# antarcticrainforest/seabreeze_param

Measured on AMD Instinct MI355X. Metric: grid-points/sec for sea_breeze_diag on N2560x1920 global grid; achieved HBM GB/s, higher is better.
Workload: dtype f64; 1 GPU; seabreeze_diag generic flavour, N1280 (2560x1920) global grid, nz=56, fp64 (BASELINE.json configs[2]); stream=torch's current stream (torch and the library share one HIP runtime), plan_cache=stored, nx=2560, ny=1920, nz=56, search_halo=16, parallelism=latband1, variant=default, comm=none, multi_rank_rccl=unmeasured on hardware so far (one GPU per box in the build pool)

## Files before the change

seabreeze_param_amd/csrc/sb_capi.hip:

```cpp
#include "../../include/seabreeze_hip.h"
#include "sb_launch.hpp"

#include <dlfcn.h>
#include <rccl/rccl.h>

#include <algorithm>
#include <chrono>
#include <cmath>
#include <condition_variable>
#include <functional>
#include <mutex>
#include <thread>
#include <cstdio>
#include <cstdlib>
#include <cstring>
#include <string>
#include <vector>

namespace {

thread_local std::string g_err;

struct DevBuf {
    void *p = nullptr;
    size_t cap = 0;
};

}

class HostPool {
  public:
    explicit HostPool(int n) {
        for (int i = 0; i < n; ++i) workers_.emplace_back([this] { loop(); });
    }
    ~HostPool() {
        { std::lock_guard<std::mutex> g(m_); quit_ = true; }
        cv_.notify_all();
        for (auto &t : workers_) t.join();
    }
    void run(int n, const std::function<void(int)> &fn) {
        if (n <= 0) return;
        {
            std::lock_guard<std::mutex> g(m_);
            fn_ = &fn; next_ = 0; total_ = n; done_ = 0;
            ++epoch_;
        }
        cv_.notify_all();
        work();
        std::unique_lock<std::mutex> lk(m_);
        done_cv_.wait(lk, [this] { return done_ == total_; });
        fn_ = nullptr;
    }
    int threads() const { return (int)workers_.size() + 1; }

  private:
    void work() {
        for (;;) {
            int i;
            const std::function<void(int)> *f;
            {
                std::lock_guard<std::mutex> g(m_);
                if (!fn_ || next_ >= total_) return;
                i = next_++;
                f = fn_;
            }
            (*f)(i);
            {
                std::lock_guard<std::mutex> g(m_);
                if (++done_ == total_) done_cv_.notify_all();
            }
        }
    }
    void loop() {
        unsigned long seen = 0;
        for (;;) {
            {
                std::unique_lock<std::mutex> lk(m_);
                cv_.wait(lk, [&] { return quit_ || epoch_ != seen; });
                if (quit_) return;
                seen = epoch_;
            }
            work();
        }
    }
    std::vector<std::thread> workers_;
    std::mutex m_;
    std::condition_variable cv_, done_cv_;
    const std::function<void(int)> *fn_ = nullptr;
    int next_ = 0, total_ = 0, done_ = 0;
    unsigned long epoch_ = 0;
    bool quit_ = false;
};

enum { SB_TICKET_WORDS = 2 };

struct DiagStream {
    bool active = false;
    HostPool *pool = nullptr;
    int nlons = 0, nlats = 0, esz = 0;
    DevBuf z, sd, cdist, ws, wd, thc, p1, theta, v, u, out;
    void *pin_in[2] = {nullptr, nullptr};
    void *pin_out[2] = {nullptr, nullptr};
    size_t pin_in_cap = 0, pin_out_cap = 0;
    hipEvent_t ev_in[2] = {nullptr, nullptr}, ev_out[2] = {nullptr, nullptr};
    long steps = 0;
    double host_copy_s = 0.0, enqueue_s = 0.0, wait_s = 0.0;
};

struct sb_ctx {
    int device = 0;
    hipStream_t stream = nullptr;
    std::string err;
    int radius_hint = 16;
    int ncu = 256;
    int ncu_dev = 256;
    int static_sigma = 0;
    bool stats_valid = false;
    int host_depth = 0;
    int no_fold = 0;
    int no_plan_cache = 0;
    int no_wide_strip = 0;
    int band_late_wind = 0;
    const void *stats_sigma = nullptr;
    int stats_dims[4] = {0, 0, 0, 0};
    int stats_ngathered = 0;
    int rep_launches = 0, rep_rccl = 0, rep_groups = 0, rep_copies = 0;
    DevBuf t0, bandbits, clsbits, tiles, vecs, nws, nwd, coastbits, tile_list, seg_list, stamps, jobcopy, plan;
    DevBuf umbits;
    int plan_key[8] = {0, 0, 0, 0, 0, 0, 0, 0};
    const void *plan_bits = nullptr;
    int call_seq = 0, plan_use = 0;
    bool segs_built = false;
    int tiles_n = 0, tiles_strip = -1, flag_parity = 0;
    int *last_flags = nullptr;
    Moments *partials = nullptr;
    unsigned int *ticket = nullptr;
    void *stats = nullptr;
    int *counters = nullptr;
    int *seg_count = nullptr;
    std::vector<unsigned char> dist_key, dist_hv;
    bool dist_ordered = false;
    double dist_maxstep = 0.0;
    hipStream_t dist_upload_stream = nullptr;
    std::vector<DevBuf> stage;
    Geo last_g{};
    int last_tiles = 0;
    bool have_last = false;
    const Moments *gathered = nullptr;
    int ngathered = 0;
    std::vector<hipEvent_t> prof_ev;
    std::vector<unsigned> prof_mask;
    int prof_calls = 0, prof_max = 0;
    hipStream_t aux_stream = nullptr;
    hipEvent_t ev_fork = nullptr, ev_join = nullptr, ev_mom = nullptr;
    Moments *band_moments_out = nullptr;
    int band_geo = 0;
    DevBuf band_mom;
    void *rccl_lib = nullptr;
    void *comm = nullptr;
    int rank = 0, nranks = 1;
    DiagStream ds;
};

namespace {

int fail(sb_ctx *c, int code, const std::string &msg) {
    if (c) c->err = msg; else g_err = msg;
    return code;
}

int hipfail(sb_ctx *c, hipError_t e, const char *what) {
    return fail(c, SB_ERR_HIP, std::string(what) + ": " + hipGetErrorString(e));
}

#define HIPCHK(c, call)                                         \
    do {                                                        \
        hipError_t e__ = (call);                                \
// ... 6 lines not shown
    b.p = nullptr;
    b.cap = 0;
    hipError_t e = hipMalloc(&b.p, bytes);
    if (e != hipSuccess) return fail(c, SB_ERR_ALLOC, std::string("hipMalloc: ") + hipGetErrorString(e));
    b.cap = bytes;
    return SB_OK;
}

template <typename T>
Geo make_geo(int nx, int ny, int h, int bnd, int rows) {
    Geo g;
    g.nx = nx; g.ny = ny; g.h = h;
    g.nxh = nx + 2 * h; g.nyh = ny + 2 * h;
    g.nw = (g.nxh + 63) / 64;
    g.bnd = bnd; g.rows = rows;
    g.band = 0;
    return g;
}

int pick_halo(const sb_ctx *c) {
    int r = c->radius_hint;
    if (r <= 8) return 8;
    if (r <= 16) return 16;
    if (r <= 24) return 24;
    return SB_MAX_LDS_HALO;
}

template <typename T>
static bool strip_kernel_runs(const sb_ctx *c, int nx, int rows) {
    const int H = pick_halo(c);
    int tx, ty;
    if (H > 16) return sizeof(T) == 4 && !c->no_wide_strip && sb_strip32_shape(nx, rows, &tx, &ty);
    return sb_strip_shape(nx, rows, &tx, &ty);
}

template <typename T>
static bool reuse_stats(const sb_ctx *c, const T *sigma, int nx, int ny, int halo) {
    return c->static_sigma && c->host_depth == 0 && c->stats_valid && c->stats_sigma == (const void *)sigma && c->stats_dims[0] == nx &&
           c->stats_dims[1] == ny && c->stats_dims[2] == halo && c->stats_dims[3] == (int)sizeof(T) &&
           c->stats_ngathered == (c->gathered ? c->ngathered : 0);
}

template <typename T>
int run_diag(sb_ctx *c, DiagJob<T> &job, hipStream_t st, int phases = 3) {
    const Geo &g = job.g;
    const size_t ncell = (size_t)g.nxh * g.nyh;
    const size_t nbits = (size_t)g.nyh * g.nw * sizeof(uint64_t);
    int rc;
    if ((rc = ensure(c, c->bandbits, nbits))) return rc;
    if ((rc = ensure(c, c->clsbits, nbits))) return rc;
    const int H = pick_halo(c);
    int txw, tyrows, tx, ty;
    const bool strip32 = H > 16 && sizeof(T) == 4 && !c->no_wide_strip && sb_strip32_shape(g.nx, g.rows, &tx, &ty);
    const bool strip = strip32 || (H <= 16 && sb_strip_shape(g.nx, g.rows, &tx, &ty));
    const int vb = strip32 ? 2 : 1;
    if (strip) { txw = 32; tyrows = 16; }
    else {
        sb_thc_tile_shape(H > 16 ? H : 24, &txw, &tyrows);
        tx = (g.nx + txw - 1) / txw; ty = (g.rows + tyrows - 1) / tyrows;
    }
    const int Hk = strip32 ? 32 : strip ? 16 : (H > 16 ? H : 24);
    const int ntile = strip ? tx * (ty + 2 * vb) : tx * ty;
    const int nflag = ntile + 2;
    if (c->tiles.cap < (size_t)2 * nflag * sizeof(int) || c->tiles_n != nflag || c->tiles_strip != (strip ? vb : 0)) {
        if ((rc = ensure(c, c->tiles, (size_t)2 * nflag * sizeof(int)))) return rc;
        HIPCHK(c, hipMemsetAsync(c->tiles.p, 0, (size_t)2 * nflag * sizeof(int), st));
        c->tiles_n = nflag;
        c->tiles_strip = strip ? vb : 0;
        c->flag_parity = 0;
    }
    int *flags_now = (int *)c->tiles.p + (size_t)c->flag_parity * nflag;
    int *flags_next = (int *)c->tiles.p + (size_t)(1 - c->flag_parity) * nflag;
    job.thc_ty = tyrows; job.thc_ntx = tx; job.thc_nty = ty;
    job.thc_txs = txw == 32 ? 5 : 6;
    job.strip = strip32 ? 2 : strip ? 1 : 0;
    if (strip) { job.tile_sx = ty + 2 * vb; job.tile_sy = 1; job.tile_off = vb; }
    else { job.tile_sx = 1; job.tile_sy = tx; job.tile_off = 0; }
    job.bandbits = (uint64_t *)c->bandbits.p;
    job.clsbits = (uint64_t *)c->clsbits.p;
    job.stats = (const T *)c->stats;
    job.tile_nnmax = flags_now;
    job.counters = flags_now + (size_t)ntile;
    job.ticket = (int *)c->ticket;
    job.next_flags = flags_next;
    job.next_flags_n = nflag;
    if ((rc = ensure(c, c->tile_list, ((size_t)ntile + (size_t)2 * c->ncu + 2) * sizeof(int)))) return rc;
    job.tile_pad = 2 * c->ncu;
    const size_t nseg = (size_t)g.nyh * g.nw;
    const size_t seg_cap = (nseg + SB_SEG_PARTS - 1) / SB_SEG_PARTS;
    if ((rc = ensure(c, c->seg_list, seg_cap * SB_SEG_PARTS * sizeof(SbSegEntry)))) return rc;
    job.tile_list = (int *)c->tile_list.p;
    job.seg_list = (SbSegEntry *)c->seg_list.p;
    job.seg_count = c->seg_count;
    job.seg_cap = (int)seg_cap;
    job.t0_fly = (job.flavour == SB_FLAVOUR_GENERIC) ? 1 : 0;
    const bool late_wind = c->band_late_wind && c->gathered && strip && job.t0_fly && !c->no_fold;
    job.wind_final = ((phases == 3 && !c->gathered) || late_wind) ? 1 : 0;
    job.nws = job.nwd = nullptr;
    if (!job.wind_final) {
        if ((rc = ensure(c, c->nws, (size_t)g.nx * g.ny * sizeof(T)))) return rc;
        if ((rc = ensure(c, c->nwd, (size_t)g.nx * g.ny * sizeof(T)))) return rc;
        job.nws = (T *)c->nws.p;
        job.nwd = (T *)c->nwd.p;
    }
    job.t0 = nullptr;
    if (!job.t0_fly) {
        if ((rc = ensure(c, c->t0, ncell * sizeof(T)))) return rc;
        job.t0 = (T *)c->t0.p;
    }
    if ((rc = ensure(c, c->jobcopy, sizeof(DiagJob<double>)))) return rc;
    job.self = (DiagJob<T> *)c->jobcopy.p;
    job.plan = nullptr; job.plan_gen = nullptr; job.call_id = 0; job.plan_use = 0; job.seg_trust = 0;
    job.moments_out = nullptr; job.stats_ticket = nullptr; job.strip_update = 0;
    if (strip) {
        const size_t need = 64 + (size_t)c->ncu * SB_PLAN_STRIDE;
        if (c->plan.cap < need) {
            if ((rc = ensure(c, c->plan, need))) return rc;
            HIPCHK(c, hipMemsetAsync(c->plan.p, 0, need, st));
            c->plan_bits = nullptr;
        }
        if (phases & 1) {
            if (c->call_seq == 0x7fffffff) {
                HIPCHK(c, hipMemsetAsync(c->plan.p, 0, need, st));
                c->call_seq = 0;
                c->plan_bits = nullptr;
            }
            ++c->call_seq;
            const int key[8] = {g.nx, g.ny, g.h, g.bnd, g.rows, c->ncu, tx, ty | (vb << 24)};
            c->plan_use = c->plan_bits == c->bandbits.p && std::memcmp(key, c->plan_key, sizeof(key)) == 0 ? 1 : 0;
            std::memcpy(c->plan_key, key, sizeof(key));
            c->plan_bits = c->bandbits.p;
        }
        job.plan = (char *)c->plan.p + 64;
        job.plan_gen = (int *)c->plan.p;
        job.call_id = c->call_seq;
        job.plan_use = c->no_plan_cache ? 0 : c->plan_use;
    } else if (phases & 1) c->plan_bits = nullptr;
    job.stamps = nullptr;
#ifdef SB_STAMPS
    if ((rc = ensure(c, c->stamps, (size_t)4096 * SB_NSTAMP * sizeof(long long)))) return rc;
    job.stamps = (long long *)c->stamps.p;
#endif
    SbLaunchCtx lc;
    lc.stream = st;
    lc.prof = nullptr;
    lc.prof_mask = nullptr;
    if (phases == 3 && c->prof_calls < c->prof_max) {
        lc.prof_mask = &c->prof_mask[(size_t)c->prof_calls];
        lc.prof = &c->prof_ev[(size_t)SB_PROF_EVENTS * c->prof_calls++];
    }
    lc.partials = c->partials; lc.stats = c->stats;
    lc.gathered = c->gathered; lc.ngathered = c->ngathered; lc.ncu = c->ncu;
    lc.moments_out = (phases == 1) ? c->band_moments_out : nullptr;
    lc.moments_event = (phases == 1 && c->nranks > 1) ? c->ev_mom : nullptr;
    lc.stats_ticket = (int *)c->ticket + 1;
    lc.phases = phases;
    lc.reuse_stats = reuse_stats<T>(c, job.sigma, g.nx, g.ny, g.h);
    lc.no_fold = c->no_fold != 0;
    const bool strip_folds = strip && job.t0_fly && !c->no_fold;
    lc.segs_stand = strip_folds && c->gathered && c->plan_use && c->segs_built && !c->no_plan_cache;
    job.fold = 0; job.fold_partials = nullptr; job.fold_nparts = 0; job.stats_out = nullptr;
    job.lists_stand = (strip_folds && !c->gathered && phases == 3 && c->plan_use && c->segs_built && !c->no_plan_cache) ? 1 : 0;
    job.gath = nullptr; job.ngath = 0;
    int launched = 0;
    lc.launches = &launched;
    if (phases == 3) c->rep_launches = c->rep_rccl = c->rep_groups = c->rep_copies = 0;
// ... 1333 lines not shown
```

seabreeze_param_amd/csrc/sb_device.hpp:

```cpp
#pragma once
#include <hip/hip_runtime.h>
#include <stdint.h>

#define SB_WAVE 64
#define SB_NSTAMP 32

enum { SB_FLAVOUR_GENERIC = 0, SB_FLAVOUR_WRAPPER = 1 };
enum { BND_WRAPPER = 0, BND_GLOBAL = 1, BND_HALO = 2 };

struct Moments {
    double n, mean, m2, mn, mx;
};

__host__ __device__ inline Moments moments_empty() {
    Moments m;
    m.n = 0.0; m.mean = 0.0; m.m2 = 0.0;
    m.mn = 1.0e308; m.mx = -1.0e308;
    return m;
}

__host__ __device__ inline Moments moments_merge(const Moments &a, const Moments &b) {
    if (b.n == 0.0) return a;
    if (a.n == 0.0) return b;
    Moments r;
// ... 104 lines not shown
        o.mx = __shfl_down(m.mx, off);
        m = moments_merge(m, o);
    }
    return m;
}

template <int NW>
__device__ __forceinline__ Moments block_merge_w(Moments m, Moments *wpart) {
    m = wave_merge(m);
    const int lane = threadIdx.x & 63, wv = threadIdx.x >> 6;
    __syncthreads();
    if (lane == 0) wpart[wv] = m;
    __syncthreads();
    Moments r = moments_empty();
    if (threadIdx.x < SB_WAVE) {
        if (threadIdx.x < NW) r = wpart[threadIdx.x];
        r = wave_merge(r);
    }
    return r;
}
__device__ __forceinline__ Moments block_merge(Moments m, Moments *wpart) {
    return block_merge_w<SB_STATS_NT / SB_WAVE>(m, wpart);
}

template <typename T>
__device__ __forceinline__ void sigmoid_scalars(const Moments &m, T *__restrict__ stats) {
    const T var = (T)m.m2;
    const T cnt = (T)m.n;
    stats[0] = T(2) / sqrt(var / cnt);
    stats[1] = ((T)m.mx - (T)m.mn) / T(4);
    stats[2] = (T)m.mean;
    stats[3] = var;
}

#endif

struct Geo {
    int nx, ny;
    int h;
    int nxh, nyh;
    int nw;
    int bnd;
    int rows;
    int band;
};
enum { GEO_BAND_EW = 1, GEO_BAND_SOUTH = 2, GEO_BAND_NORTH = 4 };

__device__ __forceinline__ bool sb_map_cell(const Geo &g, int xs, int ys, int &X, int &Y) {
    if (g.bnd == BND_HALO) {
        if (g.band & GEO_BAND_EW) {
            int m = xs % g.nx;
            xs = m < 0 ? m + g.nx : m;
        }
        if ((g.band & GEO_BAND_SOUTH) && ys < 0) ys = 0;
        if ((g.band & GEO_BAND_NORTH) && ys >= g.ny) ys = g.ny - 1;
        X = xs + g.h;
        Y = ys + g.h;
        return X >= 0 && X < g.nxh && Y >= 0 && Y < g.nyh;
    }
    int yy = ys < 0 ? 0 : (ys >= g.ny ? g.ny - 1 : ys);
    Y = yy;
    if (g.bnd == BND_WRAPPER) {
        int m = (xs + 1) % g.nx;
        if (m < 0) m += g.nx;
        X = (m < 1 ? 1 : m) - 1;
    } else {
        int m = xs % g.nx;
        if (m < 0) m += g.nx;
        X = m;
    }
    return true;
}

struct SbSegEntry {
    uint64_t word;
    uint32_t seg, pad;
};
#define SB_PLAN_SCHED 384
#define SB_PLAN_NQ 64
#define SB_PLAN_ENT_OFF 64
#define SB_PLAN_LIST_OFF (SB_PLAN_ENT_OFF + 8 * SB_PLAN_SCHED)
#define SB_PLAN_STRIDE (SB_PLAN_LIST_OFF + 2048 * SB_PLAN_NQ)
#define SB_SEG_PARTS 64

template <typename T>
struct DiagJob {
    Geo g;
    int nz;
    int flavour;
    int tn;
    int refresh;
    T target_plev, thr_wind, thr_dir, thr_ch, thr_thc, maxdist, fill;
    const T *p, *u, *v;
    const T *theta, *mask, *z, *sigma;
    int mask_ld;
    unsigned mask_off;
    int level_rule;
    T *ws, *wd, *thc, *sb_con;
    T *out;
    T *nws, *nwd;
    int *next_flags;
    int next_flags_n;
    int wind_final;
    int t0_fly;
    T *t0;
    uint64_t *bandbits;
    uint64_t *clsbits;
    const T *stats;
    int thc_ty, thc_ntx, thc_nty;
    int thc_txs;
    int tile_sx, tile_sy, tile_off;
    int strip;
    char *plan;
    int *plan_gen;
    int call_id;
    int plan_use;
    Moments *moments_out;
    int *stats_ticket;
    int strip_update;
    int seg_trust;
    int *tile_nnmax;
    int *ticket;
    int *tile_list;
    int tile_pad;
    SbSegEntry *seg_list;
    int *seg_count;
    int seg_cap;
    const Moments *gath;
    int ngath;
    int fold;
    int lists_stand;
    const Moments *fold_partials;
    int fold_nparts;
    T *stats_out;
    DiagJob<T> *self;
    int *counters;
    long long *stamps;
};

template <typename T>
struct StripJob {
    Geo g;
    const T *theta, *z, *sigma;
    const uint64_t *clsbits, *bandbits;
    T *thc;
    int *flags;
    int ntx, nty;
    int fold, fold_nparts, ngath, seg_cap;
    int lists_stand;
    int update;
    const T *stats;
    T *stats_out;
    const Moments *fold_partials, *gath;
    SbSegEntry *seg_list;
    int *seg_count;
    const DiagJob<T> *cold;
    char *plan;
    const int *plan_gen;
    int call_id, plan_use;
    long long *stamps;
};

__device__ __forceinline__ int sb_bit(const uint64_t *bits, int nw, int X, int Y) {
    return (int)((bits[(size_t)Y * nw + (X >> 6)] >> (X & 63)) & 1ull);
}

template <typename T>
__host__ __device__ inline T sb_modulo(T a, T p) {
    T r;
    if (p > T(0) && fabs(a) < p) r = a;
    else if (p > T(0) && a >= p && a < p + p) r = a - p;
    else r = fmod(a, p);
    if ((a < T(0)) != (p < T(0))) {
        if (r == T(0)) r = -r; else r += p;
    }
    return r;
}

template <typename T>
__device__ __forceinline__ T sb_logistic_of_neg(T y) {
    return T(1) / (T(1) + exp(y));
}
template <>
__device__ __forceinline__ double sb_logistic_of_neg<double>(double y) {
    y = fmin(fmax(y, -708.0), 700.0);
    const double n = __builtin_rint(y * 1.4426950408889634);
    double r = __builtin_fma(-n, 0.6931471805599453, y);
    r = __builtin_fma(-n, 2.3190468138462996e-17, r);
    const double r2 = r * r;
    double e = __builtin_fma(r2, 2.755731922398589e-07, 2.48015873015873e-05);
    double o = __builtin_fma(r2, 2.505210838544172e-08, 2.7557319223985893e-06);
    e = __builtin_fma(e, r2, 1.388888888888889e-03);   o = __builtin_fma(o, r2, 1.984126984126984e-04);
    e = __builtin_fma(e, r2, 4.1666666666666664e-02);  o = __builtin_fma(o, r2, 8.333333333333333e-03);
    e = __builtin_fma(e, r2, 0.5);                     o = __builtin_fma(o, r2, 1.6666666666666666e-01);
    e = __builtin_fma(e, r2, 1.0);                     o = __builtin_fma(o, r2, 1.0);
    const double p = __builtin_fma(o, r, e);
    const double x = 1.0 + ldexp(p, (int)n);
    double q = __builtin_amdgcn_rcp(x);
    q = __builtin_fma(q, __builtin_fma(-x, q, 1.0), q);
    q = __builtin_fma(q, __builtin_fma(-x, q, 1.0), q);
    return q;
}

template <typename T>
__device__ __forceinline__ T sb_t0(T theta, T z, T sigma, T sd, T r) {
// ... 49 lines not shown
```

seabreeze_param_amd/csrc/sb_diag_kernels.hip:

```cpp
#include "sb_device.hpp"
#include "sb_launch.hpp"
#include "sb_scan_body.hpp"

#define STATS_NT SB_STATS_NT

__device__ __forceinline__ Moments moments_from_shifted(double c, double s1, double s2, double mn, double mx,
                                                         int cnt) {
    Moments acc = moments_empty();
    if (cnt > 0) {
        acc.n = (double)cnt;
        acc.mean = c + s1 / acc.n;
        acc.m2 = s2 - s1 * s1 / acc.n;
        acc.mn = mn;
        acc.mx = mx;
    }
    return acc;
}

__device__ __forceinline__ void store_partial(Moments acc, Moments *wpart, Moments *__restrict__ partials) {
    acc = block_merge(acc, wpart);
    if (threadIdx.x == 0) partials[blockIdx.x] = acc;
}

template <typename T>
__global__ __launch_bounds__(STATS_NT) void k_stats(const T *__restrict__ ary, int nx, int ny, int ld,
                                                    size_t off0, Moments *__restrict__ partials, int *__restrict__ ticket,
                                                    T *__restrict__ stats, Moments *__restrict__ moments_out) {
    const unsigned n = (unsigned)nx * (unsigned)ny;
    const unsigned stride = gridDim.x * STATS_NT;
    const bool flat = (ld == nx);
    const double c = (double)ary[off0];
    double s1 = 0.0, s2 = 0.0, mn = 1.0e308, mx = -1.0e308;
    int cnt = 0;
    for (unsigned base = blockIdx.x * STATS_NT + threadIdx.x; base < n; base += 8 * stride) {
        double x[8];
#pragma unroll
        for (int q = 0; q < 8; ++q) {
            const unsigned i = base + q * stride;
            x[q] = c;
            if (i < n) {
                const size_t idx = flat ? (size_t)i : (size_t)(i / (unsigned)nx) * ld + (i % (unsigned)nx);
                x[q] = (double)ary[off0 + idx];
            }
        }
#pragma unroll
        for (int q = 0; q < 8; ++q) {
            if (base + q * stride < n) {
                const double d = x[q] - c;
                s1 += d;
                s2 += d * d;
                mn = x[q] < mn ? x[q] : mn;
                mx = x[q] > mx ? x[q] : mx;
                ++cnt;
            }
        }
    }
    __shared__ Moments wpart[STATS_NT / SB_WAVE];
    __shared__ int s_last;
    const Moments mine = block_merge(moments_from_shifted(c, s1, s2, mn, mx, cnt), wpart);
    if (threadIdx.x == 0) {
        double *dst = (double *)&partials[blockIdx.x];
        const double v[5] = {mine.n, mine.mean, mine.m2, mine.mn, mine.mx};
        static_assert(sizeof(Moments) == 5 * sizeof(double), "Moments is five doubles");
        for (int i = 0; i < 5; ++i) __hip_atomic_store(dst + i, v[i], __ATOMIC_RELAXED, __HIP_MEMORY_SCOPE_AGENT);
        asm volatile("s_waitcnt vmcnt(0)" ::: "memory");
        const int t = __hip_atomic_fetch_add(ticket, 1, __ATOMIC_RELAXED, __HIP_MEMORY_SCOPE_AGENT);
        s_last = t == (int)gridDim.x - 1 ? 1 : 0;
    }
    __syncthreads();
    if (!s_last) return;
    Moments m = moments_empty();
    for (int b = threadIdx.x; b < (int)gridDim.x; b += STATS_NT) {
        const double *src = (const double *)&partials[b];
        Moments o;
        o.n = __hip_atomic_load(src + 0, __ATOMIC_RELAXED, __HIP_MEMORY_SCOPE_AGENT);
        o.mean = __hip_atomic_load(src + 1, __ATOMIC_RELAXED, __HIP_MEMORY_SCOPE_AGENT);
        o.m2 = __hip_atomic_load(src + 2, __ATOMIC_RELAXED, __HIP_MEMORY_SCOPE_AGENT);
        o.mn = __hip_atomic_load(src + 3, __ATOMIC_RELAXED, __HIP_MEMORY_SCOPE_AGENT);
        o.mx = __hip_atomic_load(src + 4, __ATOMIC_RELAXED, __HIP_MEMORY_SCOPE_AGENT);
        m = moments_merge(m, o);
    }
    __syncthreads();
// ... 163 lines not shown
            const Moments o = partials[b];
            v.n += o.n; v.mean += o.mean; v.m2 += o.m2;
            v.mn = fmin(v.mn, o.mn); v.mx = fmax(v.mx, o.mx);
        }
        const Moments m = moments_of_shifted(c, block_total_shifted<PREP_NT / SB_WAVE>(v, wpart));
        if (tid == 0) {
            if (moments_out) *moments_out = m;
            else sigmoid_scalars<T>(m, stats);
        }
        return;
    }
    if (blockIdx.x == 1) {
        if (job.strip) return;
        const int ntiles = job.thc_ntx * job.thc_nty;
        int total;
        if (ntiles <= PREP_MAXCH * PREP_NT) {
            total = block_compact(ntiles, s_cnt, s_w, [&](int t) { return job.tile_nnmax[t] != 0; },
                                  [&](int rank, int t) { job.tile_list[1 + rank] = t; });
        } else {
            const int per = (ntiles + PREP_NT - 1) / PREP_NT;
            const int t0 = tid * per, t1 = min(t0 + per, ntiles);
            int cnt = 0;
            for (int t = t0; t < t1; ++t) cnt += job.tile_nnmax[t] != 0 ? 1 : 0;
            int at = block_excl_scan(cnt, s_w, total);
            for (int t = t0; t < t1; ++t)
                if (job.tile_nnmax[t] != 0) job.tile_list[1 + at++] = t;
        }
        if (tid == 0) job.tile_list[0] = total;
        for (int i = tid; i < job.tile_pad; i += PREP_NT) job.tile_list[1 + total + i] = -1;
        return;
    }
    const int part = (int)blockIdx.x - 2;
    const unsigned nseg = (unsigned)job.g.nyh * (unsigned)job.g.nw;
    const unsigned cap = (unsigned)job.seg_cap;
    const unsigned s0 = min((unsigned)part * cap, nseg), s1 = min(s0 + cap, nseg);
    SbSegEntry *list = job.seg_list + (size_t)part * cap;
    int total;
    if (cap <= (unsigned)(PREP_MAXCH * PREP_NT)) {
        total = block_compact((int)(s1 - s0), s_cnt, s_w, [&](int i) { return job.bandbits[s0 + (unsigned)i] != 0; },
                              [&](int rank, int i) {
                                  SbSegEntry e;
                                  e.word = job.bandbits[s0 + (unsigned)i]; e.seg = s0 + (unsigned)i; e.pad = 0;
                                  list[rank] = e;
                              });
    } else {
        const unsigned per = (cap + PREP_NT - 1) / PREP_NT;
        const unsigned a0 = min(s0 + (unsigned)tid * per, s1), a1 = min(a0 + per, s1);
        int cnt = 0;
        for (unsigned sg = a0; sg < a1; ++sg) cnt += job.bandbits[sg] != 0 ? 1 : 0;
        int at = block_excl_scan(cnt, s_w, total);
        for (unsigned sg = a0; sg < a1; ++sg) {
            const uint64_t w = job.bandbits[sg];
            if (w) { SbSegEntry e; e.word = w; e.seg = sg; e.pad = 0; list[at++] = e; }
        }
    }
    if (tid == 0) job.seg_count[part] = total;
}

#define WIND_NT 256

template <typename T, bool NTL>
__device__ __forceinline__ T sb_ld(const T *p) {
    if constexpr (NTL) return __builtin_nontemporal_load(p);
    else return *p;
}

template <typename T> struct WindCfg { static constexpr int UN = SB_WIND_UN, WGS = SB_WIND_WGS_PER_CU; };
template <> struct WindCfg<float> { static constexpr int UN = SB_WIND_UN_F32, WGS = SB_WIND_WGS_PER_CU_F32; };

#ifdef SB_STAMPS_WIND
#define SB_WT(i) do { if (stl_ && job.stamps) job.stamps[(size_t)gw_ * SB_NSTAMP + (i)] = wall_clock64(); } while (0)
#else
#define SB_WT(i) do { } while (0)
#endif

template <typename T, int UN, int MODE>
__global__ __launch_bounds__(WIND_NT, WindCfg<T>::WGS) void k_wind(DiagJob<T> job) {
    constexpr bool FINAL = MODE != 0;
    const Geo g = job.g;
    const int lane = threadIdx.x & 63;
#ifdef SB_STAMPS_WIND
    const int gw_ = blockIdx.x * (WIND_NT / SB_WAVE) + (threadIdx.x >> 6);
    int nsegs_ = 0;
    bool stl_ = lane == 0;
    if (gw_ < 4096 && lane < SB_NSTAMP && job.stamps) job.stamps[(size_t)gw_ * SB_NSTAMP + lane] = 0;
#endif
    SB_WT(0);
    for (int i = blockIdx.x * WIND_NT + threadIdx.x; i < job.next_flags_n; i += gridDim.x * WIND_NT) job.next_flags[i] = 0;
    const int cnt = lane < SB_SEG_PARTS ? job.seg_count[lane] : 0;
    const int incl = sb_wave_scan_add(cnt);
    const int total = __builtin_amdgcn_readlane(incl, SB_SEG_PARTS - 1);
    const int nwaves = gridDim.x * (WIND_NT / SB_WAVE);
    const int gw = __builtin_amdgcn_readfirstlane(blockIdx.x * (WIND_NT / SB_WAVE) + (threadIdx.x >> 6));
    auto entry = [&](int e) {
        const uint64_t hit = __ballot(lane < SB_SEG_PARTS && e < incl);
        const int part = hit ? __ffsll((unsigned long long)hit) - 1 : 0;
        const int base = __shfl(incl, part) - __shfl(cnt, part);
        return job.seg_list[(size_t)part * job.seg_cap + (e < total ? e - base : 0)];
    };
    const size_t pl = (size_t)g.nx * g.ny;
    const int nz = job.nz;
    int lev1 = 0;
    if (job.flavour != SB_FLAVOUR_GENERIC) {
        T best = fabs(job.p[0] - job.target_plev);
        for (int k = 1; k < nz; ++k) {
            const T a = fabs(job.p[k] - job.target_plev);
            if (a < best) { best = a; lev1 = k; }
        }
    }
    auto segment = [&](const SbSegEntry cur) __attribute__((always_inline)) {
#ifdef SB_STAMPS_WIND
        const int sbase_ = 3 + 4 * (nsegs_ < 6 ? nsegs_ : 6);
        ++nsegs_;
        stl_ = lane == __ffsll((unsigned long long)cur.word) - 1;
        SB_WT(sbase_);
#endif
        const unsigned Y = cur.seg / (unsigned)g.nw, Xw = cur.seg - Y * (unsigned)g.nw;
        const int x = (int)(Xw * 64u) + lane - g.h, y = (int)Y - g.h;
        if (!((cur.word >> lane) & 1ull)) return;
        const size_t o = (size_t)y * g.nx + x;
        T n_thc = T(0), ws_old = T(0), wd_old = T(0);
        if constexpr (FINAL) { n_thc = job.thc[o]; ws_old = job.ws[o]; wd_old = job.wd[o]; }
        int lev = lev1;
        if (job.flavour == SB_FLAVOUR_GENERIC && job.level_rule == 0) {
            const T *pc = job.p + o;
            T best = T(0);
            for (int k0 = 0; k0 < nz; k0 += UN) {
                T d[UN];
#pragma unroll
                for (int q = 0; q < UN; ++q) {
                    const int k = k0 + q < nz ? k0 + q : nz - 1;
                    d[q] = sb_ld<T, true>(pc + (size_t)k * pl);
                }
#pragma unroll
                for (int q = 0; q < UN; ++q) {
                    const int k = k0 + q;
                    const T a = fabs(d[q] - job.target_plev);
                    if (k == 0) best = a;
                    else if (k < nz && a < best) { best = a; lev = k; }
                }
            }
        } else if (job.flavour == SB_FLAVOUR_GENERIC) {
            const T *pc = job.p + o;
            T diff = T(1000000.);
            bool done = false;
            for (int k0 = 0; k0 < nz && !done; k0 += UN) {
                T d[UN];
#pragma unroll
                for (int q = 0; q < UN; ++q) {
                    const int k = k0 + q < nz ? k0 + q : nz - 1;
                    d[q] = sb_ld<T, true>(pc + (size_t)k * pl);
                }
#pragma unroll
                for (int q = 0; q < UN; ++q) {
                    const int k = k0 + q;
                    const T a = fabs(d[q] - job.target_plev);
                    if (!done && k < nz) {
                        if (a <= diff) { lev = k; diff = a; }
                        else done = true;
                    }
                }
            }
        }
#ifdef SB_STAMPS_WIND
        asm volatile("s_waitcnt vmcnt(0)" ::: "memory");
        SB_WT(sbase_ + 1);
#endif
        const T uu = job.u[(size_t)lev * pl + o];
        const T vv = job.v[(size_t)lev * pl + o];
#ifdef SB_STAMPS_WIND
        asm volatile("s_waitcnt vmcnt(0)" ::: "memory");
        SB_WT(sbase_ + 2);
#endif
        const T n_ws = sqrt(uu * uu + vv * vv);
        const T n_wd = atan2(-uu, -vv) * T(57.2957);
        if constexpr (FINAL) {
            sb_trigger_update<T, false>(job, o, n_thc, SbCellState<T>{n_ws, n_wd, ws_old, wd_old});
        } else {
            job.nws[o] = n_ws;
            job.nwd[o] = n_wd;
        }
#ifdef SB_STAMPS_WIND
        asm volatile("s_waitcnt vmcnt(0)" ::: "memory");
        SB_WT(sbase_ + 3);
#endif
    };
    if (job.seg_trust && *job.plan_gen >= job.call_id) {
        const unsigned nseg = (unsigned)g.nyh * (unsigned)g.nw;
        for (unsigned sg = (unsigned)gw; sg < nseg; sg += (unsigned)nwaves) {
            SbSegEntry cur;
            cur.word = job.bandbits[sg]; cur.seg = sg; cur.pad = 0;
            if (cur.word) segment(cur);
        }
        return;
    }
    SB_WT(1);
    if (gw >= total) return;
    SbSegEntry ent = entry(gw);
    for (int e = gw; e < total; e += nwaves) {
        const SbSegEntry cur = ent;
        if (e + nwaves < total) ent = entry(e + nwaves);
        segment(cur);
    }
#ifdef SB_STAMPS_WIND
    stl_ = lane == 0;
#endif
    SB_WT(2);
}

template <typename T>
hipError_t sb_launch_stats(const T *ary, int nx, int ny, int ld, size_t off0, Moments *partials, T *stats,
                           Moments *moments_out, int *ticket, hipStream_t st) {
    const size_t n = (size_t)nx * ny;
    int nblk = (int)((n + (size_t)STATS_NT * 8 - 1) / ((size_t)STATS_NT * 8));
    if (nblk < 1) nblk = 1;
    if (nblk > 256) nblk = 256;
    hipLaunchKernelGGL(k_stats<T>, dim3(nblk), dim3(STATS_NT), 0, st, ary, nx, ny, ld, off0, partials, ticket, stats, moments_out);
    return hipGetLastError();
}

template <typename T>
hipError_t sb_launch_sigmoid_apply(const T *ary, T *sm, size_t n, const T *stats, hipStream_t st) {
    int nblk = (int)((n + 255) / 256);
    if (nblk > 4096) nblk = 4096;
    hipLaunchKernelGGL(k_sigmoid_apply<T>, dim3(nblk), dim3(256), 0, st, ary, sm, n, stats);
    return hipGetLastError();
}

#ifndef SB_SCAN_SPT_F32
#define SB_SCAN_SPT_F32 4
#endif
template <typename T> struct SCAN_SPT { static constexpr int value = 2; };
template <> struct SCAN_SPT<float> { static constexpr int value = SB_SCAN_SPT_F32; };

template <typename T>
static void launch_scan(const DiagJob<T> &job, int nblk, Moments *partials, bool stats, hipStream_t st) {
    const bool wr = job.flavour == SB_FLAVOUR_WRAPPER;
    if (wr && stats) hipLaunchKernelGGL((k_scan<T, SCAN_SPT<T>::value, true, true>), dim3(nblk), dim3(STATS_NT), 0, st, job, partials);
    else if (wr) hipLaunchKernelGGL((k_scan<T, SCAN_SPT<T>::value, true, false>), dim3(nblk), dim3(STATS_NT), 0, st, job, partials);
    else if (stats) hipLaunchKernelGGL((k_scan<T, SCAN_SPT<T>::value, false, true>), dim3(nblk), dim3(STATS_NT), 0, st, job, partials);
    else hipLaunchKernelGGL((k_scan<T, SCAN_SPT<T>::value, false, false>), dim3(nblk), dim3(STATS_NT), 0, st, job, partials);
}

template <typename T>
static void launch_wind(const DiagJob<T> &job, int ncu, hipStream_t st) {
    const dim3 wg(ncu * WindCfg<T>::WGS), wb(WIND_NT);
    if (job.wind_final) hipLaunchKernelGGL((k_wind<T, WindCfg<T>::UN, 1>), wg, wb, 0, st, job);
    else hipLaunchKernelGGL((k_wind<T, WindCfg<T>::UN, 0>), wg, wb, 0, st, job);
}

#define SB_EV_BEGIN(k) do { if (ev) { (void)hipEventRecord(ev[2 * (k)], st); *lc.prof_mask |= 1u << (k); } } while (0)
#define SB_EV_END(k)   do { if (ev) (void)hipEventRecord(ev[2 * (k) + 1], st); } while (0)

template <typename T>
static hipError_t launch_contrast(const DiagJob<T> &job, int H, int ncu, hipStream_t st) {
    if (job.strip == 2) return sb_launch_strip32<T>(job, ncu, st);
    return job.strip ? sb_launch_strip<T>(job, ncu, st) : sb_launch_thc<T>(job, H, ncu, st);
}

template <typename T>
hipError_t sb_launch_diag(const DiagJob<T> &job, int H, const SbLaunchCtx &lc) {
    const Geo &g = job.g;
    hipStream_t st = lc.stream;
    hipEvent_t *ev = lc.prof;
    const bool gathered = lc.gathered != nullptr;
    const bool ph1 = (lc.phases & 1) != 0, ph2 = (lc.phases & 2) != 0;
    const bool reuse = lc.reuse_stats;
    hipError_t e = hipSuccess;
    int nl = 0;
    const unsigned nseg = (unsigned)g.nyh * (unsigned)g.nw;
    int nblk = (int)((nseg + 31) / 32);
    if (nblk < 1) nblk = 1;
    if (nblk > lc.ncu) nblk = lc.ncu;
    const dim3 pg(2 + SB_SEG_PARTS), pb(PREP_NT);
    if (job.wind_final && ph1 && ph2 && !gathered) {
        SB_EV_BEGIN(SB_PROF_SCAN);
        launch_scan<T>(job, nblk, lc.partials, !reuse, st);
        SB_EV_END(SB_PROF_SCAN);
        if (job.strip && job.t0_fly && !lc.no_fold && nblk <= 1024) {
            DiagJob<T> fj = job;
            fj.fold = 1;
            fj.fold_partials = lc.partials;
            fj.fold_nparts = reuse ? 0 : nblk;
            fj.stats_out = (T *)lc.stats;
            SB_EV_BEGIN(SB_PROF_THC);
            if ((e = launch_contrast<T>(fj, H, lc.ncu, st)) != hipSuccess) return e;
            SB_EV_END(SB_PROF_THC);
            SB_EV_BEGIN(SB_PROF_WIND);
// ... 113 lines not shown
```

seabreeze_param_amd/csrc/sb_scan_body.hpp:

```cpp
#pragma once
#include "sb_device.hpp"
#ifndef SB_EAGER_PLANES
#define SB_EAGER_PLANES 0
#endif

template <typename T, int SPT, bool WR, bool ST>
__device__ __forceinline__ bool sb_scan_pass(const DiagJob<T> &job, Moments &mine, unsigned kernarg_job_off = 0) {
    constexpr bool wrapper = WR, do_stats = ST;
    constexpr int SCAN_NT = SB_STATS_NT;
    const Geo g = job.g;
    const int lane = threadIdx.x & 63, wv = threadIdx.x >> 6;
    constexpr int NWV = SCAN_NT / SB_WAVE;
    const unsigned nseg = (unsigned)g.nyh * (unsigned)g.nw;
    const unsigned nwaves = gridDim.x * NWV;
    const size_t pl = (size_t)g.nx * g.ny;
    if (blockIdx.x == 0 && threadIdx.x == 0 && job.ticket) *job.ticket = 0;
    if (blockIdx.x == 0 && job.self && threadIdx.x < sizeof(DiagJob<T>) / 4)
        ((unsigned *)job.self)[threadIdx.x] =
            ((const __attribute__((address_space(4))) unsigned *)__builtin_amdgcn_kernarg_segment_ptr())[kernarg_job_off / 4 + threadIdx.x];
    const double c = do_stats ? (double)job.sigma[(size_t)g.h * g.nxh + g.h] : 0.0;
    double s1 = 0.0, s2 = 0.0, mn = 1.0e308, mx = -1.0e308;
    int cnt = 0;

    const unsigned w0 = __builtin_amdgcn_readfirstlane(blockIdx.x * NWV + wv);
    const unsigned unw = (unsigned)g.nw;
    unsigned Yc = w0 / unw, Xc = w0 - Yc * unw;
    const unsigned dY = nwaves / unw, dX = nwaves - dY * unw;
    const unsigned nxh = (unsigned)g.nxh, unx = (unsigned)g.nx;

    struct Trip {
        T sg[SPT], mk[SPT], ws[SPT], wd[SPT];
        uint64_t old;
        unsigned Y[SPT], W[SPT];
    };
    bool plane_changed = false;
    static_assert(2 * SPT <= SB_WAVE, "two lanes per segment of a trip");
    auto issue = [&](unsigned s0, Trip &t) {
        {
            const unsigned seg = s0 + (unsigned)(lane >> 1) * nwaves;
            const uint64_t *plane = (lane & 1) ? job.clsbits : job.bandbits;
            t.old = plane[(lane < 2 * SPT && seg < nseg) ? seg : 0u];
        }
#pragma unroll
        for (int q = 0; q < SPT; ++q) {
            const unsigned seg = s0 + q * nwaves;
            t.Y[q] = Yc;
            t.W[q] = Xc;
            const int X = (int)(Xc * 64u) + lane;
            const int xi = X - g.h, yi = (int)Yc - g.h;
            const bool in = seg < nseg && X < g.nxh;
            const bool interior = in && xi >= 0 && xi < g.nx && yi >= 0 && yi < g.ny;
            const unsigned idx = in ? Yc * nxh + (unsigned)X : 0u;
            t.mk[q] = job.mask[job.mask_off + (in ? Yc * (unsigned)job.mask_ld + (unsigned)X : 0u)];
            t.sg[q] = T(0); t.ws[q] = T(0); t.wd[q] = T(0);
            if (do_stats) t.sg[q] = job.sigma[idx];
            if (wrapper) {
                const unsigned o = (interior && yi < g.rows) ? (unsigned)yi * unx + (unsigned)xi : 0u;
                t.ws[q] = job.ws[o];
                t.wd[q] = job.wd[o];
            }
            Yc += dY; Xc += dX;
            if (Xc >= unw) { Xc -= unw; Yc += 1; }
        }
    };
    auto process = [&](unsigned s0, const Trip &t) {
        uint64_t now = t.old;
#pragma unroll
        for (int q = 0; q < SPT; ++q) {
            const unsigned seg = s0 + q * nwaves;
            if (seg >= nseg) break;
            const int X = (int)(t.W[q] * 64u) + lane, xi = X - g.h, yi = (int)t.Y[q] - g.h;
            const bool in = X < g.nxh;
            const bool interior = in && xi >= 0 && xi < g.nx && yi >= 0 && yi < g.ny;
            if (do_stats && interior) {
                const double x = (double)t.sg[q], d = x - c;
                s1 += d;
                s2 = __builtin_fma(d, d, s2);
                mn = fmin(mn, x);
                mx = fmax(mx, x);
                ++cnt;
            }
            const bool cls = in && (t.mk[q] >= T(0));
            const bool band = interior && yi < g.rows && !(fabs(t.mk[q]) > job.maxdist);
            const uint64_t wc = __ballot(cls);
            const uint64_t wb = __ballot(band);
            if ((lane >> 1) == q) {
                now = (lane & 1) ? wc : wb;
                if (SB_EAGER_PLANES || now != t.old) ((lane & 1) ? job.clsbits : job.bandbits)[seg] = now;
            }
            if (wb) {
                const int txs = job.thc_txs, tw = 1 << txs;
                const int xi0 = (int)(t.W[q] * 64u) - g.h;
                const int tA = xi0 >> txs;
                int lo = ((tA + lane) << txs) - xi0, hi = lo + tw;
                lo = lo < 0 ? 0 : lo;
                hi = hi > 64 ? 64 : hi;
                if (lane <= (64 >> txs) && lo < hi) {
                    const uint64_t m = (hi - lo == 64 ? ~0ull : ((1ull << (hi - lo)) - 1ull)) << lo;
                    if (wb & m) job.tile_nnmax[(tA + lane) * job.tile_sx + (yi / job.thc_ty) * job.tile_sy + job.tile_off] = 1;
// ... 31 lines not shown
```

Baseline: 42.17 billion grid-points/s.

## Replace static wind segment striding with sharded atomic ticket work stealing

The wind kernel's loop over band segments changes from a fixed stride of nwaves to dynamic scheduling. Each wave draws its next entry from one of 16 atomic ticket counters, sharded by workgroup and spaced 64 ints apart to avoid contention on a single address. The draw is issued during the final pressure-level load chunk so its latency overlaps the memory loads. The tickets are reset in the scan kernel, and the stamp instrumentation now also records line counts. The aim is to balance uneven per-segment work across waves, at the cost of extra atomics and more complex control flow.

```diff
diff --git a/seabreeze_param_amd/csrc/sb_capi.hip b/seabreeze_param_amd/csrc/sb_capi.hip
--- a/seabreeze_param_amd/csrc/sb_capi.hip
+++ b/seabreeze_param_amd/csrc/sb_capi.hip
@@ -92,7 +92,7 @@
     bool quit_ = false;
 };
 
-enum { SB_TICKET_WORDS = 2 };
+enum { SB_TICKET_WIND = SB_WIND_TICKET_STRIDE, SB_TICKET_WORDS = SB_TICKET_WIND + SB_WIND_SHARDS * SB_WIND_TICKET_STRIDE };
 
 struct DiagStream {
     bool active = false;
@@ -265,6 +265,7 @@
     job.tile_nnmax = flags_now;
     job.counters = flags_now + (size_t)ntile;
     job.ticket = (int *)c->ticket;
+    job.wind_tickets = (int *)c->ticket + SB_TICKET_WIND;
     job.next_flags = flags_next;
     job.next_flags_n = nflag;
     if ((rc = ensure(c, c->tile_list, ((size_t)ntile + (size_t)2 * c->ncu + 2) * sizeof(int)))) return rc;
diff --git a/seabreeze_param_amd/csrc/sb_device.hpp b/seabreeze_param_amd/csrc/sb_device.hpp
--- a/seabreeze_param_amd/csrc/sb_device.hpp
+++ b/seabreeze_param_amd/csrc/sb_device.hpp
@@ -210,6 +210,8 @@
 #define SB_PLAN_LIST_OFF (SB_PLAN_ENT_OFF + 8 * SB_PLAN_SCHED)
 #define SB_PLAN_STRIDE (SB_PLAN_LIST_OFF + 2048 * SB_PLAN_NQ)
 #define SB_SEG_PARTS 64
+#define SB_WIND_SHARDS 16
+#define SB_WIND_TICKET_STRIDE 64
 
 template <typename T>
 struct DiagJob {
@@ -249,6 +251,7 @@
     int seg_trust;
     int *tile_nnmax;
     int *ticket;
+    int *wind_tickets;
     int *tile_list;
     int tile_pad;
     SbSegEntry *seg_list;
diff --git a/seabreeze_param_amd/csrc/sb_diag_kernels.hip b/seabreeze_param_amd/csrc/sb_diag_kernels.hip
--- a/seabreeze_param_amd/csrc/sb_diag_kernels.hip
+++ b/seabreeze_param_amd/csrc/sb_diag_kernels.hip
@@ -1,3 +1,4 @@
+#include <type_traits>
 #include "sb_device.hpp"
 #include "sb_launch.hpp"
 #include "sb_scan_body.hpp"
@@ -327,7 +328,8 @@
 #ifdef SB_STAMPS_WIND
     const int gw_ = blockIdx.x * (WIND_NT / SB_WAVE) + (threadIdx.x >> 6);
     int nsegs_ = 0;
-    bool stl_ = lane == 0;
+    long long lines_ = 0;
+    bool stl_ = lane == 0 && gw_ < 4096;
     if (gw_ < 4096 && lane < SB_NSTAMP && job.stamps) job.stamps[(size_t)gw_ * SB_NSTAMP + lane] = 0;
 #endif
     SB_WT(0);
@@ -353,64 +355,93 @@
             if (a < best) { best = a; lev1 = k; }
         }
     }
-    auto segment = [&](const SbSegEntry cur) __attribute__((always_inline)) {
+    const int nsh = (int)gridDim.x < SB_WIND_SHARDS ? (int)gridDim.x : SB_WIND_SHARDS;
+    const int shard = (int)blockIdx.x % nsh;
+    int *const tickets = job.wind_tickets + shard * SB_WIND_TICKET_STRIDE;
+    const int drawn0 = (((int)gridDim.x - shard + nsh - 1) / nsh) * (WIND_NT / SB_WAVE);
+    auto ticket_entry = [&](int j) { return ((j >> 2) * nsh + shard) * 4 + (j & 3); };
+    static_assert(WIND_NT / SB_WAVE == 4, "a shard's tickets go by workgroups of four waves");
+    int tk = 0;
+    auto segment = [&](const SbSegEntry cur, auto draw_tag, SbSegEntry &next, bool &more) __attribute__((always_inline)) {
+        constexpr bool DRAW = decltype(draw_tag)::value;
+        const int first = __builtin_amdgcn_readfirstlane(__ffsll((unsigned long long)cur.word) - 1);
 #ifdef SB_STAMPS_WIND
         const int sbase_ = 3 + 4 * (nsegs_ < 6 ? nsegs_ : 6);
+        if (nsegs_ < 7) {
+            const int per = 128 / (int)sizeof(T);
+            int nl = 0;
+            for (int q = 0; q < 64 / per; ++q) nl += ((cur.word >> (q * per)) & ((1ull << per) - 1ull)) != 0;
+            lines_ |= (long long)nl << (3 * nsegs_);
+        }
         ++nsegs_;
-        stl_ = lane == __ffsll((unsigned long long)cur.word) - 1;
+        stl_ = lane == first && gw_ < 4096;
         SB_WT(sbase_);
 #endif
         const unsigned Y = cur.seg / (unsigned)g.nw, Xw = cur.seg - Y * (unsigned)g.nw;
         const int x = (int)(Xw * 64u) + lane - g.h, y = (int)Y - g.h;
-        if (!((cur.word >> lane) & 1ull)) return;
-        const size_t o = (size_t)y * g.nx + x;
+        const bool inband = (cur.word >> lane) & 1ull;
+        const size_t o = inband ? (size_t)y * g.nx + x : 0;
         T n_thc = T(0), ws_old = T(0), wd_old = T(0);
-        if constexpr (FINAL) { n_thc = job.thc[o]; ws_old = job.ws[o]; wd_old = job.wd[o]; }
         int lev = lev1;
-        if (job.flavour == SB_FLAVOUR_GENERIC && job.level_rule == 0) {
-            const T *pc = job.p + o;
-            T best = T(0);
-            for (int k0 = 0; k0 < nz; k0 += UN) {
-                T d[UN];
-#pragma unroll
-                for (int q = 0; q < UN; ++q) {
-                    const int k = k0 + q < nz ? k0 + q : nz - 1;
-                    d[q] = sb_ld<T, true>(pc + (size_t)k * pl);
+        auto draw = [&]() {
+            if (lane == first) tk = __hip_atomic_fetch_add(tickets, 1, __ATOMIC_RELAXED, __HIP_MEMORY_SCOPE_AGENT);
+        };
+        if (inband) {
+            if constexpr (FINAL) { n_thc = job.thc[o]; ws_old = job.ws[o]; wd_old = job.wd[o]; }
+            const bool whole = job.flavour == SB_FLAVOUR_GENERIC && job.level_rule == 0;
+            if constexpr (DRAW) { if (!whole) draw(); }
+            if (whole) {
+                const T *pc = job.p + o;
+                T best = T(0);
+                for (int k0 = 0; k0 < nz; k0 += UN) {
+                    T d[UN];
+                    if constexpr (DRAW) { if (k0 + UN >= nz) draw(); }
+#pragma unroll
+                    for (int q = 0; q < UN; ++q) {
+                        const int k = k0 + q < nz ? k0 + q : nz - 1;
+                        d[q] = sb_ld<T, true>(pc + (size_t)k * pl);
+                    }
+#pragma unroll
+                    for (int q = 0; q < UN; ++q) {
+                        const int k = k0 + q;
+                        const T a = fabs(d[q] - job.target_plev);
+                        if (k == 0) best = a;
+                        else if (k < nz && a < best) { best = a; lev = k; }
+                    }
                 }
-#pragma unroll
-                for (int q = 0; q < UN; ++q) {
-                    const int k = k0 + q;
-                    const T a = fabs(d[q] - job.target_plev);
-                    if (k == 0) best = a;
-                    else if (k < nz && a < best) { best = a; lev = k; }
-                }
-            }
-        } else if (job.flavour == SB_FLAVOUR_GENERIC) {
-            const T *pc = job.p + o;
-            T diff = T(1000000.);
-            bool done = false;
-            for (int k0 = 0; k0 < nz && !done; k0 += UN) {
-                T d[UN];
-#pragma unroll
-                for (int q = 0; q < UN; ++q) {
-                    const int k = k0 + q < nz ? k0 + q : nz - 1;
-                    d[q] = sb_ld<T, true>(pc + (size_t)k * pl);
-                }
-#pragma unroll
-                for (int q = 0; q < UN; ++q) {
-                    const int k = k0 + q;
-                    const T a = fabs(d[q] - job.target_plev);
-                    if (!done && k < nz) {
-                        if (a <= diff) { lev = k; diff = a; }
-                        else done = true;
+            } else if (job.flavour == SB_FLAVOUR_GENERIC) {
+                const T *pc = job.p + o;
+                T diff = T(1000000.);
+                bool done = false;
+                for (int k0 = 0; k0 < nz && !done; k0 += UN) {
+                    T d[UN];
+#pragma unroll
+                    for (int q = 0; q < UN; ++q) {
+                        const int k = k0 + q < nz ? k0 + q : nz - 1;
+                        d[q] = sb_ld<T, true>(pc + (size_t)k * pl);
+                    }
+#pragma unroll
+                    for (int q = 0; q < UN; ++q) {
+                        const int k = k0 + q;
+                        const T a = fabs(d[q] - job.target_plev);
+                        if (!done && k < nz) {
+                            if (a <= diff) { lev = k; diff = a; }
+                            else done = true;
+                        }
                     }
                 }
             }
-        }
 #ifdef SB_STAMPS_WIND
-        asm volatile("s_waitcnt vmcnt(0)" ::: "memory");
-        SB_WT(sbase_ + 1);
-#endif
+            asm volatile("s_waitcnt vmcnt(0)" ::: "memory");
+            SB_WT(sbase_ + 1);
+#endif
+        }
+        if constexpr (DRAW) {
+            const int e = ticket_entry(drawn0 + __builtin_amdgcn_readlane(tk, first));
+            more = e < total;
+            next = entry(e);
+        }
+        if (!inband) return;
         const T uu = job.u[(size_t)lev * pl + o];
         const T vv = job.v[(size_t)lev * pl + o];
 #ifdef SB_STAMPS_WIND
@@ -430,25 +461,27 @@
         SB_WT(sbase_ + 3);
 #endif
     };
+    SbSegEntry ent;
+    bool more = true;
     if (job.seg_trust && *job.plan_gen >= job.call_id) {
         const unsigned nseg = (unsigned)g.nyh * (unsigned)g.nw;
         for (unsigned sg = (unsigned)gw; sg < nseg; sg += (unsigned)nwaves) {
             SbSegEntry cur;
             cur.word = job.bandbits[sg]; cur.seg = sg; cur.pad = 0;
-            if (cur.word) segment(cur);
+            if (cur.word) segment(cur, std::false_type{}, ent, more);
         }
         return;
     }
     SB_WT(1);
     if (gw >= total) return;
-    SbSegEntry ent = entry(gw);
-    for (int e = gw; e < total; e += nwaves) {
+    ent = entry(gw);
+    while (more) {
         const SbSegEntry cur = ent;
-        if (e + nwaves < total) ent = entry(e + nwaves);
-        segment(cur);
+        segment(cur, std::true_type{}, ent, more);
     }
 #ifdef SB_STAMPS_WIND
-    stl_ = lane == 0;
+    stl_ = lane == 0 && gw_ < 4096;
+    if (stl_ && job.stamps) job.stamps[(size_t)gw_ * SB_NSTAMP + SB_NSTAMP - 1] = lines_;
 #endif
     SB_WT(2);
 }
diff --git a/seabreeze_param_amd/csrc/sb_scan_body.hpp b/seabreeze_param_amd/csrc/sb_scan_body.hpp
--- a/seabreeze_param_amd/csrc/sb_scan_body.hpp
+++ b/seabreeze_param_amd/csrc/sb_scan_body.hpp
@@ -15,6 +15,7 @@
     const unsigned nwaves = gridDim.x * NWV;
     const size_t pl = (size_t)g.nx * g.ny;
     if (blockIdx.x == 0 && threadIdx.x == 0 && job.ticket) *job.ticket = 0;
+    if (blockIdx.x == 0 && threadIdx.x < SB_WIND_SHARDS && job.wind_tickets) job.wind_tickets[threadIdx.x * SB_WIND_TICKET_STRIDE] = 0;
     if (blockIdx.x == 0 && job.self && threadIdx.x < sizeof(DiagJob<T>) / 4)
         ((unsigned *)job.self)[threadIdx.x] =
             ((const __attribute__((address_space(4))) unsigned *)__builtin_amdgcn_kernarg_segment_ptr())[kernarg_job_off / 4 + threadIdx.x];
```

Result: no change. 42.00 billion grid-points/s (-0.4%).
